# yanivw12/gs2mesh

Measured on AMD Instinct MI355X. Metric: stereo-pair renders/sec + TSDF Mvoxel-updates/sec, higher is better.
Workload: dtype f32

## Files before the change

gs2mesh_amd/_lib.py:

```python
from __future__ import annotations

import ctypes as C

import numpy as np
import os

try:
    import torch
except Exception:
    torch = None

_HERE = os.path.dirname(os.path.abspath(__file__))
LIB_PATH = os.path.join(_HERE, "libgs2mesh_amd.so")

vp = C.c_void_p
i32 = C.c_int
i64 = C.c_int64
f32 = C.c_float
f64 = C.c_double


class Camera(C.Structure):
    _fields_ = [("width", C.c_int32), ("height", C.c_int32), ("tanfovx", f32), ("tanfovy", f32),
                ("viewmatrix", f32 * 16), ("projmatrix", f32 * 16), ("campos", f32 * 3)]
# ... 73 lines not shown
    "gs2m_photo_loss_scratch_bytes": (i64, [i32, i32, i32]),
    "gs2m_photo_loss_forward": (i32, [i32, i32, i32, vp, vp, f32, vp, i64, vp, vp, vp, vp]),
    "gs2m_photo_loss_backward": (i32, [i32, i32, i32, vp, vp, vp, f32, vp, vp, vp]),
    "gs2m_adam_step": (i32, [i32, C.POINTER(AdamSegment), vp, i64, vp]),
    "gs2m_densify_stats": (i32, [i32, vp, vp, vp, vp, vp, vp]),
    "gs2m_mask_preprocess": (i32, [i32, i32, i32, C.POINTER(vp), C.POINTER(vp), i32, i32, i32, i32, C.POINTER(vp), vp, vp]),
    "gs2m_tsdf_create": (i32, [C.POINTER(vp), f64, f64, i32, i32, i32, i64, i32]),
    "gs2m_tsdf_destroy": (i32, [vp]),
    "gs2m_tsdf_reset": (i32, [vp, vp]),
    "gs2m_tsdf_integrate": (i32, [vp, vp, vp, vp, i32, i32, f64, f64, f64, f64, C.POINTER(f64), f64, f64, f64, vp]),
    "gs2m_tsdf_integrate_batch": (i32, [vp, i32, C.POINTER(vp), C.POINTER(vp), C.POINTER(vp), i32, i32, f64, f64, f64, f64,
                                        C.POINTER(f64), f64, f64, f64, vp]),
    "gs2m_tsdf_set_stage_timing": (i32, [vp, i32]),
    "gs2m_tsdf_stage_times": (i32, [vp, vp, C.POINTER(f64), C.POINTER(i64)]),
    "gs2m_tsdf_status": (i32, [vp, vp, C.POINTER(i64), C.POINTER(i64), C.POINTER(i32)]),
    "gs2m_tsdf_download": (i32, [vp, vp, i64, vp, vp, vp, vp]),
    "gs2m_tsdf_block_keys": (i32, [vp, i64, vp, vp]),
    "gs2m_tsdf_flags_device": (i32, [vp, vp, vp]),
    "gs2m_tsdf_pack_sum": (i32, [vp, vp, i64, vp, vp]),
    "gs2m_tsdf_unpack_sum": (i32, [vp, vp, i64, vp, i32, vp]),
    "gs2m_tsdf_pack": (i32, [vp, vp, i64, i32, vp, vp, vp]),
    "gs2m_tsdf_extract_mesh": (i32, [vp, vp, C.POINTER(i64), C.POINTER(i64)]),
    "gs2m_tsdf_mesh_copy": (i32, [vp, vp, vp, vp, vp, vp]),
    "gs2m_mesh_cluster": (i32, [i32, vp, i64, vp, vp, vp, C.POINTER(i64)]),
    "gs2m_mesh_vertex_normals": (i32, [i32, vp, i64, vp, i64, vp, vp, vp]),
    "gs2m_tsdf_replace": (i32, [vp, vp, i64, i32, vp, vp, vp]),
    "gs2m_tsdf_map_bytes": (i64, [C.POINTER(C.c_int32), i32]),
    "gs2m_tsdf_block_map": (i32, [vp, C.POINTER(C.c_int32), C.POINTER(C.c_int32), i32, i32, i64, i64, i32, vp, vp]),
    "gs2m_tsdf_map_keys": (i32, [vp, C.POINTER(C.c_int32), C.POINTER(C.c_int32), i32, vp, vp, i64, C.POINTER(C.c_uint8), vp]),
    "gs2m_tsdf_unpack": (i32, [vp, vp, i64, i32, vp, vp, i32, vp]),
# ... 130 lines not shown
```

gs2mesh_amd/csrc/tsdf_api.hip:

```cpp
#include <math.h>
#include <stdio.h>
#include <string.h>

#include <mutex>
#include <vector>

#include "../../include/gs2mesh_amd.h"
#include "device_memory.h"
#include "tsdf_common.h"
#include "tsdf_internal.h"

struct gs2m_tsdf {
    int device = 0;
    double voxel_length = 0, sdf_trunc = 0, unit_length = 0;
    int color_type = 1, resolution = 16, stride = 4;
    TsdfVolume V;
    struct {
        DeviceBuffer<float> tsdf, weight;
        DeviceBuffer<unsigned> rgb, stamp, touched, counters;
        DeviceBuffer<int> block_keys, hash_vals;
        DeviceBuffer<unsigned char> halo;
        DeviceBuffer<unsigned long long> hash_keys, fmask, totals;
    } vol;
    unsigned frame_id = 0;
    PinnedBuffer<unsigned> h_counters;
    PinnedBuffer<unsigned long long> h_totals;
    int n_cu = 256;
    DeviceBuffer<unsigned char> d_mc;
    const McDevTables* mc() const { return reinterpret_cast<const McDevTables*>(d_mc.get()); }
    DeviceBuffer<unsigned> d_blk_tris;
    DeviceBuffer<unsigned long long> d_ntri;
    DeviceBuffer<double> mesh_v, mesh_c;
    DeviceBuffer<int> mesh_e;
    DeviceBuffer<int> mesh_tri;
    int64_t mesh_nv = 0, mesh_nt = 0;
    ScratchArena mesh_scratch;
    int timing = 0;
// ... 39 lines not shown
    TsdfVolume& V = t->V;
    if (whole_pool) {
        GS2M_HIPCHK(hipMemsetAsync(V.tsdf, 0, sizeof(float) * (size_t)V.max_blocks * GS2M_TSDF_VOX, st));
        GS2M_HIPCHK(hipMemsetAsync(V.weight, 0, sizeof(float) * (size_t)V.max_blocks * GS2M_TSDF_VOX, st));
        if (V.rgb) GS2M_HIPCHK(hipMemsetAsync(V.rgb, 0, sizeof(unsigned) * 3 * (size_t)V.max_blocks * GS2M_TSDF_VOX, st));
        GS2M_HIPCHK(hipMemsetAsync(V.halo, 0, (size_t)V.max_blocks, st));
    } else if (keep_first < 0) {
        gs2m_launch_tsdf_clear_used(st, V);
    } else {
        gs2m_launch_tsdf_clear_from(st, V, (unsigned)keep_first);
    }
    GS2M_HIPCHK(hipMemsetAsync(V.hash_keys, 0xff, sizeof(unsigned long long) * (size_t)V.hash_cap, st));
    GS2M_HIPCHK(hipMemsetAsync(V.hash_vals, 0xff, sizeof(int) * (size_t)V.hash_cap, st));
    GS2M_HIPCHK(hipMemsetAsync(V.stamp, 0, sizeof(unsigned) * (size_t)V.hash_cap, st));
    GS2M_HIPCHK(hipMemsetAsync(V.fmask, 0, sizeof(unsigned long long) * (size_t)V.hash_cap, st));
    GS2M_HIPCHK(hipMemsetAsync(V.counters, 0, sizeof(unsigned) * 4, st));
    GS2M_HIPCHK(hipMemsetAsync(V.totals, 0, sizeof(unsigned long long), st));
    return 0;
}

static int init_volume(gs2m_tsdf* t, int64_t max_blocks) {
    memset(&t->V, 0, sizeof(t->V));
    TsdfVolume& V = t->V;
    V.max_blocks = (unsigned)max_blocks;
    unsigned cap = 1024;
    while ((uint64_t)cap < 2ull * (uint64_t)max_blocks) cap <<= 1;
    V.hash_cap = cap;
    V.has_color = t->color_type == GS2M_TSDF_COLOR_RGB8;
    const size_t nvox = (size_t)max_blocks * GS2M_TSDF_VOX, nb = (size_t)max_blocks;
    auto& o = t->vol;
    if (o.tsdf.reserve_exact(nvox) || o.weight.reserve_exact(nvox) || (V.has_color && o.rgb.reserve_exact(3 * nvox)) ||
        o.block_keys.reserve_exact(3 * nb) || o.halo.reserve_exact(nb) || o.hash_keys.reserve_exact(cap) ||
        o.hash_vals.reserve_exact(cap) || o.stamp.reserve_exact(cap) || o.touched.reserve_exact(cap) || o.fmask.reserve_exact(cap) ||
        t->d_bframes.reserve_exact(GS2M_TSDF_MAX_BATCH) || t->h_bframes.reserve(GS2M_TSDF_MAX_BATCH * gs2m_tsdf::kRing) ||
        o.counters.reserve_exact(4) || o.totals.reserve_exact(1) || t->d_mc.reserve_exact(gs2m_mc_tables_bytes()) ||
        t->d_blk_tris.reserve_exact(nb) || t->d_ntri.reserve_exact(1) || t->h_counters.reserve(4) || t->h_totals.reserve(1)) {
        gs2m_set_error("gs2m_tsdf_create: out of device memory for %lld blocks (%.1f MiB)", (long long)max_blocks,
                       (double)nvox * 20.0 / 1048576.0);
        return 1;
    }
    V.tsdf = o.tsdf.get();
    V.weight = o.weight.get();
    V.rgb = o.rgb.get();
    V.block_keys = o.block_keys.get();
    V.halo = o.halo.get();
    V.hash_keys = o.hash_keys.get();
    V.hash_vals = o.hash_vals.get();
    V.stamp = o.stamp.get();
    V.touched = o.touched.get();
    V.fmask = o.fmask.get();
    V.counters = o.counters.get();
    V.totals = o.totals.get();
    std::vector<unsigned char> tab(gs2m_mc_tables_bytes());
    if (!gs2m_mc_tables_fill(tab.data()) ||
        hipMemcpy(t->d_mc.get(), tab.data(), tab.size(), hipMemcpyHostToDevice) != hipSuccess) {
        gs2m_set_error("gs2m_tsdf_create: marching-cubes table generation failed");
        return 1;
    }
    if (zero_state(t, (hipStream_t)0, true)) return 1;
    GS2M_HIPCHK(hipStreamSynchronize((hipStream_t)0));
    return 0;
}

extern "C" int gs2m_tsdf_create(gs2m_tsdf** out, double voxel_length, double sdf_trunc, int color_type,
                                int volume_unit_resolution, int depth_sampling_stride, int64_t max_blocks,
                                int device) {
    if (!out) {
// ... 157 lines not shown
            const int i = f0 + k;
            if (!depth[i] || (t->V.has_color && !color[i])) {
                gs2m_set_error("gs2m_tsdf_integrate_batch: frame %d has a NULL image", i);
                return 1;
            }
            const unsigned char* m = mask ? mask[i] : nullptr;
            if (fill_frame(t, hb[k].f, width, height, fx, fy, cx, cy, extrinsics_w2c + 16 * (size_t)i, depth_scale, depth_trunc,
                           min_depth, m != nullptr))
                return 1;
            hb[k].depth = depth[i];
            hb[k].color = color ? color[i] : nullptr;
            hb[k].mask = m;
        }
        GS2M_HIPCHK(hipMemcpyAsync(t->d_bframes.get(), hb, sizeof(TsdfBatchFrame) * nf, hipMemcpyHostToDevice, st));
        GS2M_HIPCHK(hipEventRecord(t->ring_done[slot], st));
        GS2M_HIPCHK(hipMemsetAsync(t->V.counters + 1, 0, sizeof(unsigned), st));
        GS2M_HIPCHK(hipMemsetAsync(t->V.counters + 3, 0, sizeof(unsigned), st));
        {
            StageTimer tm(t->events, t->timing != 0, st, 0, "gs2m:tsdf_touch_batch", nf);
            gs2m_launch_tsdf_touch_batch(st, t->V, hb[0].f, nf, t->d_bframes.get(), t->d_tiles.get());
        }
        {
            StageTimer tm(t->events, t->timing != 0, st, 1, "gs2m:tsdf_integrate_batch", nf);
            gs2m_launch_tsdf_integrate_batch(st, t->n_cu, t->V, t->d_bframes.get(), t->d_tiles.get());
        }
    }
    return 0;
}

extern "C" int gs2m_tsdf_set_stage_timing(gs2m_tsdf* t, int enable) {
    if (!t) {
        gs2m_set_error("null handle");
// ... 17 lines not shown
                                int* overflow) {
    if (!t) {
        gs2m_set_error("null handle");
        return 1;
    }
    hipStream_t st = (hipStream_t)stream;
    GS2M_HIPCHK(hipMemcpyAsync(t->h_counters.get(), t->V.counters, sizeof(unsigned) * 4, hipMemcpyDeviceToHost, st));
    GS2M_HIPCHK(hipMemcpyAsync(t->h_totals.get(), t->V.totals, sizeof(unsigned long long), hipMemcpyDeviceToHost, st));
    GS2M_HIPCHK(hipStreamSynchronize(st));
    GS2M_HIPCHK(hipGetLastError());
    unsigned nb = t->h_counters.get()[0];
    if (nb > t->V.max_blocks) nb = t->V.max_blocks;
    if (n_blocks) *n_blocks = nb;
    if (block_updates) *block_updates = (int64_t)t->h_totals.get()[0];
    if (overflow) *overflow = (int)t->h_counters.get()[2];
    return 0;
}

extern "C" int gs2m_tsdf_flags_device(gs2m_tsdf* t, uint32_t* flags_dev, gs2m_stream stream) {
    if (!t || !flags_dev) {
        gs2m_set_error("gs2m_tsdf_flags_device: NULL argument");
        return 1;
    }
    GS2M_HIPCHK(hipSetDevice(t->device));
    GS2M_HIPCHK(hipMemcpyAsync(flags_dev, t->V.counters + 2, sizeof(unsigned), hipMemcpyDeviceToDevice, (hipStream_t)stream));
    return 0;
}

extern "C" int gs2m_tsdf_block_keys(gs2m_tsdf* t, int64_t n, int32_t* keys, gs2m_stream stream) {
    if (!t || (n > 0 && !keys) || n < 0 || n > (int64_t)t->V.max_blocks) {
// ... 410 lines not shown
```

gs2mesh_amd/csrc/tsdf_common.h:

```cpp
#pragma once
#include "platform.h"

#define GS2M_TSDF_RES 16
#define GS2M_TSDF_VOX 4096
#define GS2M_TSDF_EMPTY 0xffffffffffffffffull
#define GS2M_TSDF_KEY_BIAS (1 << 20)

struct TsdfVolume {
    float* tsdf;
    float* weight;
    unsigned* rgb;
    int* block_keys;
    unsigned char* halo;
    unsigned long long* hash_keys;
    int* hash_vals;
    unsigned* stamp;
    unsigned* touched;
    unsigned long long* fmask;
    unsigned* counters;
    unsigned long long* totals;
    unsigned hash_cap;
    unsigned max_blocks;
    int has_color;
};

struct alignas(16) TsdfFrame {
    float E[12];
    double pose[12];
    double fx, fy, cx, cy;
    double unit_length, sdf_trunc, depth_trunc;
    float fx_f, fy_f, cx_f, cy_f, fx_inv_f, fy_inv_f;
    float voxel_length_f, half_voxel_length_f, sdf_trunc_f, sdf_trunc_inv_f;
    float Es02, Es12, Es22;
    float safe_w, safe_h;
    float depth_scale_f, min_depth_f;
    float depth_trunc_up_f;
    int W, H, stride, nx, ny;
    unsigned frame_id;
    int use_mask, use_min;
};

struct TsdfBatchFrame {
    TsdfFrame f;
    const float* depth;
    const unsigned char* color;
    const unsigned char* mask;
};
#define GS2M_TSDF_MAX_BATCH 64
#define GS2M_TSDF_TILE 8
#define GS2M_TSDF_TILES(n) (((n) + GS2M_TSDF_TILE - 1) / GS2M_TSDF_TILE)
#define GS2M_TSDF_CULL_MAX_TILES 48

#define GS2M_TSDF_VINDEX(x, y, z) (((((z) >> 2) * 16 + ((x) >> 2) * 4 + ((y) >> 2)) * 64) + ((z)&3) * 16 + ((x)&3) * 4 + ((y)&3))

GS2M_DEVICE unsigned long long tsdf_pack_key(int bx, int by, int bz) {
    return ((unsigned long long)(unsigned)(bx + GS2M_TSDF_KEY_BIAS) << 42) |
           ((unsigned long long)(unsigned)(by + GS2M_TSDF_KEY_BIAS) << 21) |
           (unsigned long long)(unsigned)(bz + GS2M_TSDF_KEY_BIAS);
}
GS2M_DEVICE void tsdf_unpack_key(unsigned long long key, int& bx, int& by, int& bz) {
    bx = (int)((key >> 42) & 0x1fffffull) - GS2M_TSDF_KEY_BIAS;
    by = (int)((key >> 21) & 0x1fffffull) - GS2M_TSDF_KEY_BIAS;
// ... 15 lines not shown
```

gs2mesh_amd/csrc/tsdf_internal.h:

```cpp
#pragma once
#include "api_check.h"
#include "tsdf_common.h"

void gs2m_launch_tsdf_touch(hipStream_t st, const TsdfVolume& V, const TsdfFrame& f, const float* depth,
                            const unsigned char* mask);
void gs2m_launch_tsdf_integrate(hipStream_t st, int n_wg, const TsdfVolume& V, const TsdfFrame& f,
                                const float* depth, const unsigned char* color, const unsigned char* mask);
void gs2m_launch_tsdf_touch_batch(hipStream_t st, const TsdfVolume& V, const TsdfFrame& f, int n_frames,
                                  const TsdfBatchFrame* frames, float* tiles);
void gs2m_launch_tsdf_integrate_batch(hipStream_t st, int n_wg, const TsdfVolume& V, const TsdfBatchFrame* frames, const float* tiles);
void gs2m_launch_tsdf_clear_used(hipStream_t st, const TsdfVolume& V);
void gs2m_launch_tsdf_pack(hipStream_t st, unsigned n, const TsdfVolume& V, const int* keys, int form, float* buf, long long* ibuf);
void gs2m_launch_tsdf_unpack(hipStream_t st, unsigned n, const TsdfVolume& V, const int* keys, int form, const float* buf,
                             const long long* ibuf, int halo);
void gs2m_launch_tsdf_clear_from(hipStream_t st, const TsdfVolume& V, unsigned first);
void gs2m_launch_tsdf_clear_gap(hipStream_t st, const TsdfVolume& V, unsigned upto);
void gs2m_launch_tsdf_owned_keys(hipStream_t st, unsigned n, const TsdfVolume& V, int* keys);
void gs2m_launch_tsdf_block_map(hipStream_t st, const TsdfVolume& V, const int* lo, const int* dim, unsigned char* cells, unsigned n_cells,
                                unsigned flags, unsigned win_hash, int rank, unsigned frames_local, unsigned frames_base);
void gs2m_launch_tsdf_map_keys(hipStream_t st, const int* lo, const int* dim, unsigned char* cells, unsigned n_cells, int* keys, unsigned max_keys);
struct McDevTables;
size_t gs2m_mc_tables_bytes();
bool gs2m_mc_tables_fill(void* host_buf);
void gs2m_launch_mc_count(hipStream_t st, const TsdfVolume& V, const McDevTables* T, unsigned n_blocks,
                          unsigned* blk_tris, unsigned long long* n_total);
// ... 18 lines not shown
```

gs2mesh_amd/csrc/tsdf_kernels.h:

```cpp
#pragma once
#include "tsdf_common.h"


GS2M_DEVICE void tsdf_cam_point(const TsdfFrame& f, float p0, float p1, float p2, float& pc0, float& pc1, float& pc2) {
    pc0 = f.E[0] * p0 + f.E[1] * p1 + f.E[2] * p2 + f.E[3] * 1.f;
    pc1 = f.E[4] * p0 + f.E[5] * p1 + f.E[6] * p2 + f.E[7] * 1.f;
    pc2 = f.E[8] * p0 + f.E[9] * p1 + f.E[10] * p2 + f.E[11] * 1.f;
}
GS2M_DEVICE void tsdf_z_step(const TsdfFrame& f, float& pc0, float& pc1, float& pc2) {
    pc0 += f.Es02;
    pc1 += f.Es12;
    pc2 += f.Es22;
}
GS2M_DEVICE int tsdf_project(const TsdfFrame& f, float pc0, float pc1, float pc2, int& u, int& v) {
    if (pc2 <= 0) return -1;
    const float u_f = pc0 * f.fx_f / pc2 + f.cx_f + 0.5f;
    const float v_f = pc1 * f.fy_f / pc2 + f.cy_f + 0.5f;
    if (!(u_f >= 0.0001f && u_f < f.safe_w && v_f >= 0.0001f && v_f < f.safe_h)) return -1;
    u = (int)u_f;
    v = (int)v_f;
    return v * f.W + u;
}
GS2M_DEVICE float tsdf_distance_multiplier(const TsdfFrame& f, int u, int v) {
    const float xx = (u - f.cx_f) * f.fx_inv_f;
// ... 20 lines not shown
    return d > 0.0f && sdf > -f.sdf_trunc_f;
}
GS2M_DEVICE unsigned tsdf_gather_rgb(const unsigned char* __restrict__ color, int pix, int last_pix) {
    const unsigned char* c = color + 3 * (size_t)pix;
    return pix < last_pix ? gs2m_load_u32_unaligned(c) : ((unsigned)c[0] | ((unsigned)c[1] << 8) | ((unsigned)c[2] << 16));
}
GS2M_DEVICE void tsdf_update_mean(float& t, float& w, float tnew) {
    t = (t * w + tnew) / (w + 1.0f);
    w = w + 1.0f;
}
GS2M_DEVICE void tsdf_update_rgb(unsigned& c0, unsigned& c1, unsigned& c2, unsigned rgbp) {
    c0 += rgbp & 0xffu;
    c1 += (rgbp >> 8) & 0xffu;
    c2 += (rgbp >> 16) & 0xffu;
}
GS2M_DEVICE float tsdf_block_centres(const TsdfFrame& f, unsigned long long key, int tid, float* s_p0, float* s_p1) {
    int bx, by, bz;
    tsdf_unpack_key(key, bx, by, bz);
    const double ox = (double)bx * f.unit_length, oy = (double)by * f.unit_length, oz = (double)bz * f.unit_length;
    if (tid < 16) s_p0[tid] = (float)(f.half_voxel_length_f + f.voxel_length_f * tid + ox);
    else if (tid < 32) s_p1[tid - 16] = (float)(f.half_voxel_length_f + f.voxel_length_f * (tid - 16) + oy);
    return (float)(f.half_voxel_length_f + oz);
}

GS2M_DEVICE unsigned tsdf_find_or_insert(const TsdfVolume& V, unsigned long long key, int bx, int by, int bz) {
    const unsigned mask = V.hash_cap - 1u;
    unsigned h = tsdf_hash(key) & mask;
    for (unsigned probe = 0; probe < V.hash_cap; ++probe, h = (h + 1u) & mask) {
        unsigned long long k = V.hash_keys[h];
        if (k == key) return h;
        if (k == GS2M_TSDF_EMPTY) {
            const unsigned long long prev = atomicCAS(&V.hash_keys[h], GS2M_TSDF_EMPTY, key);
            if (prev == GS2M_TSDF_EMPTY) {
                const unsigned slot = atomicAdd(&V.counters[0], 1u);
                if (slot < V.max_blocks) {
                    V.block_keys[3 * (size_t)slot] = bx;
// ... 303 lines not shown
        }
#pragma unroll
        for (int s = 1; s < GS2M_TSDF_TILE; s <<= 1) {
            const float o = gs2m_shfl_xor(m, s);
            if (o > m) m = o;
        }
        if ((lane & (GS2M_TSDF_TILE - 1)) == 0 && x < f.W) out[x / GS2M_TSDF_TILE] = m;
    }
}

GS2M_KERNEL void __launch_bounds__(256)
k_tsdf_touch_batch(TsdfVolume V, const TsdfBatchFrame* __restrict__ frames, unsigned n_touch, float* __restrict__ tiles, int tiles_x,
                   int tiles_y, unsigned map_wg_x) {
    __shared__ TouchStage stage_all[4];
    const TsdfBatchFrame& bf = frames[blockIdx.y];
    if (blockIdx.x < n_touch) {
        tsdf_touch_body(V, bf.f, bf.depth, bf.mask, stage_all, (int)blockIdx.y);
    } else {
        const unsigned m = blockIdx.x - n_touch, ty = m / map_wg_x;
        tsdf_depth_tiles_body(bf, tiles + ((size_t)blockIdx.y * tiles_y + ty) * tiles_x, (int)(m - ty * map_wg_x), (int)ty);
    }
}

GS2M_DEVICE bool tsdf_pass_live(const TsdfFrame& f0, const float4* __restrict__ e4, const float* __restrict__ tiles, int tiles_x,
                                float xa, float xb, float ya, float yb, float z0) {
    const float4 r0 = e4[0], r1 = e4[1], r2 = e4[2];
    const float vl = f0.voxel_length_f, zspan = 15.0f * vl;
    const float ax = fmaxf(fabsf(xa), fabsf(xb)), ay = fmaxf(fabsf(ya), fabsf(yb)), az = fabsf(z0) + zspan + vl;
    const float S = fmaxf(fmaxf(fabsf(r0.x) * ax + fabsf(r0.y) * ay + fabsf(r0.z) * az + fabsf(r0.w),
                                fabsf(r1.x) * ax + fabsf(r1.y) * ay + fabsf(r1.z) * az + fabsf(r1.w)),
                          fabsf(r2.x) * ax + fabsf(r2.y) * ay + fabsf(r2.z) * az + fabsf(r2.w));
    const float eps = S * (1.0f / 262144.0f);
    const float bx = r0.x * xa + r0.y * ya + r0.z * z0 + r0.w, by = r1.x * xa + r1.y * ya + r1.z * z0 + r1.w,
                bz = r2.x * xa + r2.y * ya + r2.z * z0 + r2.w;
    const float dx[3] = {r0.x * (xb - xa), r0.y * (yb - ya), r0.z * zspan};
    const float dy[3] = {r1.x * (xb - xa), r1.y * (yb - ya), r1.z * zspan};
    const float dz[3] = {r2.x * (xb - xa), r2.y * (yb - ya), r2.z * zspan};
    float cx[8], cy[8], cz[8], zmin = bz;
// ... 17 lines not shown
        vmax = fmaxf(vmax, v);
        mag += fabsf(u) + fabsf(v);
    }
    if (!(mag < 1e9f)) return true;
    const float au = fmaxf(fabsf(umin), fabsf(umax)), av = fmaxf(fabsf(vmin), fabsf(vmax));
    const float k = eps / zl, rnd = 1.0f / 1048576.0f;
    const float mu = 1.0f + k * (fabsf(f0.fx_f) + au) + rnd * (au + fabsf(f0.cx_f) + 1.0f);
    const float mv = 1.0f + k * (fabsf(f0.fy_f) + av) + rnd * (av + fabsf(f0.cy_f) + 1.0f);
    if (!(mu < 1e6f && mv < 1e6f)) return true;
    const float x0 = fmaxf(floorf(umin + f0.cx_f - mu), 0.0f), x1 = fminf(ceilf(umax + f0.cx_f + mu), (float)(f0.W - 1));
    const float y0 = fmaxf(floorf(vmin + f0.cy_f - mv), 0.0f), y1 = fminf(ceilf(vmax + f0.cy_f + mv), (float)(f0.H - 1));
    if (x0 > x1 || y0 > y1) return false;
    const int tx0 = (int)x0 / GS2M_TSDF_TILE, tx1 = (int)x1 / GS2M_TSDF_TILE, ty0 = (int)y0 / GS2M_TSDF_TILE, ty1 = (int)y1 / GS2M_TSDF_TILE;
    if ((tx1 - tx0 + 1) * (ty1 - ty0 + 1) > GS2M_TSDF_CULL_MAX_TILES) return true;
    float dmax = 0.0f;
    for (int ty = ty0; ty <= ty1; ty += 4) {
        for (int tx = tx0; tx <= tx1; tx += 4) {
            float d[16];
#pragma unroll
            for (int i = 0; i < 4; ++i) {
                const float* __restrict__ row = tiles + (size_t)(ty + i < ty1 ? ty + i : ty1) * tiles_x;
#pragma unroll
                for (int j = 0; j < 4; ++j) d[4 * i + j] = row[tx + j < tx1 ? tx + j : tx1];
            }
#pragma unroll
            for (int i = 0; i < 16; ++i)
                if (d[i] > dmax) dmax = d[i];
        }
    }
    if (!(dmax > 0.0f)) return false;
    const float zlow = zl - vl;
    return !(dmax - zlow <= -f0.sdf_trunc_f);
}

GS2M_KERNEL void __launch_bounds__(256)
k_tsdf_integrate_batch(TsdfVolume V, const TsdfBatchFrame* __restrict__ frames, const float* __restrict__ tiles) {
    __shared__ float s_p0[16], s_p1[16];
    const int tid = (int)threadIdx.x;
    const int lane = tid & 63, wave = tid >> 6;
    const int lz = lane >> 4, lx = (lane >> 2) & 3, ly = lane & 3;
    __shared__ unsigned s_it;
    const unsigned n_touched = V.counters[1] * 4u;
    const TsdfFrame& f0 = frames[0].f;
    for (;;) {
        __syncthreads();
        if (tid == 0) s_it = atomicAdd(&V.counters[3], 1u);
        __syncthreads();
        const unsigned it = s_it;
        if (it >= n_touched) break;
        const int xq = (int)(it & 3u);
        const unsigned h = V.touched[it >> 2];
        const unsigned long long key = V.hash_keys[h];
        const int slot = V.hash_vals[h];
        const unsigned long long fm = V.fmask[h];
        if (slot < 0) continue;
        const float p2 = tsdf_block_centres(f0, key, tid, s_p0, s_p1);
        __syncthreads();
        const float p0 = s_p0[4 * xq + lx], p1 = s_p1[4 * wave + ly];
        const int vi0 = (xq * 4 + wave) * 64 + lane;
        constexpr int VS = 16 * 64;
        float* bt = V.tsdf + (size_t)slot * GS2M_TSDF_VOX;
        float* bw = V.weight + (size_t)slot * GS2M_TSDF_VOX;
        unsigned* bc = V.rgb + (size_t)slot * 3 * GS2M_TSDF_VOX;
        bool live = false;
        if ((fm >> lane) & 1ull) {
            const int tiles_x = GS2M_TSDF_TILES(f0.W), tiles_y = GS2M_TSDF_TILES(f0.H);
            live = tsdf_pass_live(f0, reinterpret_cast<const float4*>(frames[lane].f.E), tiles + (size_t)lane * tiles_y * tiles_x, tiles_x,
                                  s_p0[4 * xq], s_p0[4 * xq + 3], s_p1[4 * wave], s_p1[4 * wave + 3], p2);
        }
        const unsigned long long fm_live = fm & gs2m_ballot(live ? 1 : 0);
        float w[4], t[4];
        unsigned c0[4], c1[4], c2[4];
#pragma unroll
        for (int j = 0; j < 4; ++j) {
            w[j] = t[j] = 0.0f;
            c0[j] = c1[j] = c2[j] = 0u;
            if (fm_live != 0ull) {
                w[j] = bw[vi0 + VS * j];
                t[j] = bt[vi0 + VS * j];
                if (V.has_color) {
                    c0[j] = bc[vi0 + VS * j];
                    c1[j] = bc[GS2M_TSDF_VOX + vi0 + VS * j];
                    c2[j] = bc[2 * GS2M_TSDF_VOX + vi0 + VS * j];
                }
            }
// ... 85 lines not shown
                if (todo == 0ull) break;
            }
            apply(A);
        }
#pragma unroll
        for (int j = 0; j < 4; ++j) {
            if (fm_live == 0ull) continue;
            bw[vi0 + VS * j] = w[j];
            bt[vi0 + VS * j] = t[j];
            if (V.has_color) {
                bc[vi0 + VS * j] = c0[j];
                bc[GS2M_TSDF_VOX + vi0 + VS * j] = c1[j];
                bc[2 * GS2M_TSDF_VOX + vi0 + VS * j] = c2[j];
            }
        }
        if (tid == 0 && xq == 0) atomicAdd(&V.totals[0], (unsigned long long)gs2m_popc64(fm));
    }
}

GS2M_KERNEL void __launch_bounds__(256)
k_tsdf_clear_fmask(TsdfVolume V) {
    const unsigned n = V.counters[1];
    for (unsigned i = blockIdx.x * 256u + threadIdx.x; i < n; i += gridDim.x * 256u) V.fmask[V.touched[i]] = 0ull;
}

GS2M_KERNEL void __launch_bounds__(256)
k_tsdf_clear_used(TsdfVolume V) {
    unsigned n = V.counters[0];
    if (n > V.max_blocks) n = V.max_blocks;
    const float4 z = {0.f, 0.f, 0.f, 0.f};
    for (unsigned slot = blockIdx.x; slot < n; slot += gridDim.x) {
        float4* t4 = reinterpret_cast<float4*>(V.tsdf + (size_t)slot * GS2M_TSDF_VOX);
        float4* w4 = reinterpret_cast<float4*>(V.weight + (size_t)slot * GS2M_TSDF_VOX);
        for (int i = (int)threadIdx.x; i < GS2M_TSDF_VOX / 4; i += 256) {
            t4[i] = z;
            w4[i] = z;
        }
        if (V.has_color) {
// ... 223 lines not shown
```

gs2mesh_amd/csrc/tsdf_kernels.hip:

```cpp
#include "tsdf_kernels.h"
#include "tsdf_extract.h"
#include "mesh_kernels.h"
#include "tsdf_internal.h"
#include <math.h>

void gs2m_launch_tsdf_touch(hipStream_t st, const TsdfVolume& V, const TsdfFrame& f, const float* depth,
                            const unsigned char* mask) {
    const int n = f.nx * f.ny;
    GS2M_LAUNCH(k_tsdf_touch, dim3((n + 255) / 256), dim3(256), 0, st, V, f, depth, mask);
    GS2M_LAUNCH(k_tsdf_compact, dim3((V.hash_cap + 1023u) / 1024u), dim3(1024), 0, st, V, f.frame_id);
}
void gs2m_launch_tsdf_integrate(hipStream_t st, int n_wg, const TsdfVolume& V, const TsdfFrame& f,
                                const float* depth, const unsigned char* color, const unsigned char* mask) {
    GS2M_LAUNCH(k_tsdf_integrate, dim3(n_wg), dim3(256), 0, st, V, f, depth, color, mask);
}
void gs2m_launch_tsdf_touch_batch(hipStream_t st, const TsdfVolume& V, const TsdfFrame& f, int n_frames,
                                  const TsdfBatchFrame* frames, float* tiles) {
    const int n = f.nx * f.ny;
    const int tiles_x = GS2M_TSDF_TILES(f.W), tiles_y = GS2M_TSDF_TILES(f.H);
    const unsigned n_touch = (unsigned)((n + 255) / 256), map_wg_x = (unsigned)((f.W + 1023) / 1024);
    GS2M_LAUNCH(k_tsdf_touch_batch, dim3(n_touch + map_wg_x * (unsigned)tiles_y, n_frames), dim3(256), 0, st, V, frames, n_touch, tiles, tiles_x,
                tiles_y, map_wg_x);
    GS2M_LAUNCH(k_tsdf_compact, dim3((V.hash_cap + 1023u) / 1024u), dim3(1024), 0, st, V, 0u);
}
void gs2m_launch_tsdf_integrate_batch(hipStream_t st, int n_cu, const TsdfVolume& V, const TsdfBatchFrame* frames, const float* tiles) {
    GS2M_LAUNCH(k_tsdf_integrate_batch, dim3(n_cu * 6), dim3(256), 0, st, V, frames, tiles);
    GS2M_LAUNCH(k_tsdf_clear_fmask, dim3(16), dim3(256), 0, st, V);
}
void gs2m_launch_tsdf_clear_used(hipStream_t st, const TsdfVolume& V) {
    GS2M_LAUNCH(k_tsdf_clear_used, dim3(2048), dim3(256), 0, st, V);
}
void gs2m_launch_tsdf_pack(hipStream_t st, unsigned n, const TsdfVolume& V, const int* keys, int form, float* buf, long long* ibuf) {
    if (form == GS2M_XF_SUM_PACKED) GS2M_LAUNCH(k_tsdf_pack<GS2M_XF_SUM_PACKED>, dim3(n), dim3(256), 0, st, V, keys, buf, ibuf);
    else if (form == GS2M_XF_RAW_F32) GS2M_LAUNCH(k_tsdf_pack<GS2M_XF_RAW_F32>, dim3(n), dim3(256), 0, st, V, keys, buf, ibuf);
    else GS2M_LAUNCH(k_tsdf_pack<GS2M_XF_SUM_F32>, dim3(n), dim3(256), 0, st, V, keys, buf, ibuf);
}
void gs2m_launch_tsdf_unpack(hipStream_t st, unsigned n, const TsdfVolume& V, const int* keys, int form, const float* buf,
                             const long long* ibuf, int halo) {
    if (form == GS2M_XF_SUM_PACKED) GS2M_LAUNCH(k_tsdf_unpack<GS2M_XF_SUM_PACKED>, dim3(n), dim3(256), 0, st, V, keys, buf, ibuf, halo);
    else if (form == GS2M_XF_RAW_F32) GS2M_LAUNCH(k_tsdf_unpack<GS2M_XF_RAW_F32>, dim3(n), dim3(256), 0, st, V, keys, buf, ibuf, halo);
    else GS2M_LAUNCH(k_tsdf_unpack<GS2M_XF_SUM_F32>, dim3(n), dim3(256), 0, st, V, keys, buf, ibuf, halo);
}
// ... 93 lines not shown
```

gs2mesh_amd/integration.py:

```python
from __future__ import annotations

import ctypes as C
import enum

import numpy as np

from . import _lib
from ._lib import _is_torch, _ptr, _stream_of

try:
    import torch
except Exception:
    torch = None


class TSDFVolumeColorType(enum.IntEnum):
    NoColor = 0
    RGB8 = 1
    Gray32 = 2


class PinholeCameraIntrinsic:
    def __init__(self, width, height, fx, fy, cx, cy):
        self.width, self.height = int(width), int(height)
# ... 153 lines not shown
        if len(self._keep) > 64:
            self.status(stream)

    def status(self, stream=None, raise_on_overflow=True):
        nb, bu, ov = C.c_int64(0), C.c_int64(0), C.c_int(0)
        _lib.check(self._lib.gs2m_tsdf_status(self._h, stream or C.c_void_p(0), C.byref(nb), C.byref(bu),
                                              C.byref(ov)), self._lib)
        self._keep.clear()
        if ov.value and raise_on_overflow:
            what = [n for b, n in ((1, "block pool exhausted (raise max_blocks)"), (2, "hash table full"),
                                   (4, "block index out of the +-2^20 range"),
                                   (8, "a voxel did not fit the packed exchange form (weight > 1023: use payload='f32')")) if ov.value & b]
            raise RuntimeError("TSDF volume overflow: " + ", ".join(what))
        return int(nb.value), int(bu.value), int(ov.value)

    def set_stage_timing(self, enable=True):
        _lib.check(self._lib.gs2m_tsdf_set_stage_timing(self._h, int(bool(enable))), self._lib)

    def stage_times(self, stream=None):
        ms = (C.c_double * 2)()
        cnt = (C.c_int64 * 2)()
        _lib.check(self._lib.gs2m_tsdf_stage_times(self._h, stream or C.c_void_p(0), ms, cnt), self._lib)
        return {name: (ms[i], cnt[i]) for i, name in enumerate(_lib.TSDF_STAGES)}

    @property
    def num_blocks(self):
        return self.status()[0]

    @property
    def voxel_updates(self):
# ... 115 lines not shown
```

include/gs2mesh_amd.h:

```cpp
#ifndef GS2MESH_AMD_H
#define GS2MESH_AMD_H

#include <stddef.h>
#include <stdint.h>

#ifdef __cplusplus
extern "C" {
#endif

#define GS2M_VERSION 600

typedef void* gs2m_stream;


int gs2m_version(void);
const char* gs2m_last_error(void);


typedef struct gs2m_raster gs2m_raster;

enum {
    GS2M_OPT_EXACT_TILE_CULL = 1,
    GS2M_OPT_BLEND_VARIANT = 2,
    GS2M_OPT_DEBUG_SYNC = 3,
// ... 120 lines not shown
int gs2m_tsdf_integrate(gs2m_tsdf* t, const float* depth, const uint8_t* color,
                        const uint8_t* mask, int width, int height, double fx, double fy,
                        double cx, double cy, const double* extrinsic_w2c, double depth_scale,
                        double depth_trunc, double min_depth, gs2m_stream stream);

int gs2m_tsdf_integrate_batch(gs2m_tsdf* t, int n_frames, const float* const* depth, const uint8_t* const* color,
                              const uint8_t* const* mask, int width, int height, double fx, double fy, double cx,
                              double cy, const double* extrinsics_w2c, double depth_scale, double depth_trunc,
                              double min_depth, gs2m_stream stream);

int gs2m_tsdf_set_stage_timing(gs2m_tsdf* t, int enable);
int gs2m_tsdf_stage_times(gs2m_tsdf* t, gs2m_stream stream, double* total_ms, int64_t* launches);

int gs2m_tsdf_status(gs2m_tsdf* t, gs2m_stream stream, int64_t* n_blocks,
                     int64_t* block_updates, int* overflow);

int gs2m_tsdf_flags_device(gs2m_tsdf* t, uint32_t* flags_dev, gs2m_stream stream);

int gs2m_tsdf_download(gs2m_tsdf* t, gs2m_stream stream, int64_t n, int32_t* keys,
                       float* tsdf, float* weight, uint32_t* rgb_sum);

int gs2m_tsdf_block_keys(gs2m_tsdf* t, int64_t n, int32_t* keys, gs2m_stream stream);

int gs2m_tsdf_pack_sum(gs2m_tsdf* t, const int32_t* keys, int64_t n, float* buf, gs2m_stream stream);
int gs2m_tsdf_unpack_sum(gs2m_tsdf* t, const int32_t* keys, int64_t n, const float* buf, int halo,
                         gs2m_stream stream);

#define GS2M_TSDF_MAP_HEADER_BYTES 32
int64_t gs2m_tsdf_map_bytes(const int32_t* dim, int world);
int gs2m_tsdf_block_map(gs2m_tsdf* t, const int32_t* lo, const int32_t* dim, int rank, int world, int64_t frames_local,
// ... 103 lines not shown
```

Baseline: 4268.

## Split TSDF batch integration into a frame-liveness plan pass and integrate pass

Adds a planning kernel that, per touched block and x-quarter, evaluates frame liveness culling in parallel across 16 lanes per frame-chunk and writes a compact plan item (key, slot, per-wave live masks). The integrate kernel reads the plan, skips block quarters with no live frames before computing centres, and drops its own per-lane culling and the separate fmask-clear kernel. Counter resets move from host memsets into the touch kernel, and the tile max scan uses unaligned 4-wide loads. It adds an extra kernel launch and a plan buffer of four items per hash slot, plus a diagnostic plan-count API.

```diff
diff --git a/gs2mesh_amd/_lib.py b/gs2mesh_amd/_lib.py
--- a/gs2mesh_amd/_lib.py
+++ b/gs2mesh_amd/_lib.py
@@ -111,6 +111,7 @@
     "gs2m_tsdf_set_stage_timing": (i32, [vp, i32]),
     "gs2m_tsdf_stage_times": (i32, [vp, vp, C.POINTER(f64), C.POINTER(i64)]),
     "gs2m_tsdf_status": (i32, [vp, vp, C.POINTER(i64), C.POINTER(i64), C.POINTER(i32)]),
+    "gs2m_tsdf_plan_counts": (i32, [vp, vp, C.POINTER(i64), C.POINTER(i64)]),
     "gs2m_tsdf_download": (i32, [vp, vp, i64, vp, vp, vp, vp]),
     "gs2m_tsdf_block_keys": (i32, [vp, i64, vp, vp]),
     "gs2m_tsdf_flags_device": (i32, [vp, vp, vp]),
diff --git a/gs2mesh_amd/csrc/tsdf_api.hip b/gs2mesh_amd/csrc/tsdf_api.hip
--- a/gs2mesh_amd/csrc/tsdf_api.hip
+++ b/gs2mesh_amd/csrc/tsdf_api.hip
@@ -21,6 +21,7 @@
         DeviceBuffer<int> block_keys, hash_vals;
         DeviceBuffer<unsigned char> halo;
         DeviceBuffer<unsigned long long> hash_keys, fmask, totals;
+        DeviceBuffer<TsdfPlanItem> plan;
     } vol;
     unsigned frame_id = 0;
     PinnedBuffer<unsigned> h_counters;
@@ -90,8 +91,8 @@
     GS2M_HIPCHK(hipMemsetAsync(V.hash_vals, 0xff, sizeof(int) * (size_t)V.hash_cap, st));
     GS2M_HIPCHK(hipMemsetAsync(V.stamp, 0, sizeof(unsigned) * (size_t)V.hash_cap, st));
     GS2M_HIPCHK(hipMemsetAsync(V.fmask, 0, sizeof(unsigned long long) * (size_t)V.hash_cap, st));
-    GS2M_HIPCHK(hipMemsetAsync(V.counters, 0, sizeof(unsigned) * 4, st));
-    GS2M_HIPCHK(hipMemsetAsync(V.totals, 0, sizeof(unsigned long long), st));
+    GS2M_HIPCHK(hipMemsetAsync(V.counters, 0, sizeof(unsigned) * GS2M_TSDF_COUNTERS, st));
+    GS2M_HIPCHK(hipMemsetAsync(V.totals, 0, sizeof(unsigned long long) * GS2M_TSDF_TOTALS, st));
     return 0;
 }
 
@@ -109,8 +110,9 @@
         o.block_keys.reserve_exact(3 * nb) || o.halo.reserve_exact(nb) || o.hash_keys.reserve_exact(cap) ||
         o.hash_vals.reserve_exact(cap) || o.stamp.reserve_exact(cap) || o.touched.reserve_exact(cap) || o.fmask.reserve_exact(cap) ||
         t->d_bframes.reserve_exact(GS2M_TSDF_MAX_BATCH) || t->h_bframes.reserve(GS2M_TSDF_MAX_BATCH * gs2m_tsdf::kRing) ||
-        o.counters.reserve_exact(4) || o.totals.reserve_exact(1) || t->d_mc.reserve_exact(gs2m_mc_tables_bytes()) ||
-        t->d_blk_tris.reserve_exact(nb) || t->d_ntri.reserve_exact(1) || t->h_counters.reserve(4) || t->h_totals.reserve(1)) {
+        o.counters.reserve_exact(GS2M_TSDF_COUNTERS) || o.totals.reserve_exact(GS2M_TSDF_TOTALS) ||
+        o.plan.reserve_exact(4 * (size_t)cap) || t->d_mc.reserve_exact(gs2m_mc_tables_bytes()) ||
+        t->d_blk_tris.reserve_exact(nb) || t->d_ntri.reserve_exact(1) || t->h_counters.reserve(4) || t->h_totals.reserve(GS2M_TSDF_TOTALS)) {
         gs2m_set_error("gs2m_tsdf_create: out of device memory for %lld blocks (%.1f MiB)", (long long)max_blocks,
                        (double)nvox * 20.0 / 1048576.0);
         return 1;
@@ -127,6 +129,7 @@
     V.fmask = o.fmask.get();
     V.counters = o.counters.get();
     V.totals = o.totals.get();
+    V.plan = o.plan.get();
     std::vector<unsigned char> tab(gs2m_mc_tables_bytes());
     if (!gs2m_mc_tables_fill(tab.data()) ||
         hipMemcpy(t->d_mc.get(), tab.data(), tab.size(), hipMemcpyHostToDevice) != hipSuccess) {
@@ -314,8 +317,6 @@
         }
         GS2M_HIPCHK(hipMemcpyAsync(t->d_bframes.get(), hb, sizeof(TsdfBatchFrame) * nf, hipMemcpyHostToDevice, st));
         GS2M_HIPCHK(hipEventRecord(t->ring_done[slot], st));
-        GS2M_HIPCHK(hipMemsetAsync(t->V.counters + 1, 0, sizeof(unsigned), st));
-        GS2M_HIPCHK(hipMemsetAsync(t->V.counters + 3, 0, sizeof(unsigned), st));
         {
             StageTimer tm(t->events, t->timing != 0, st, 0, "gs2m:tsdf_touch_batch", nf);
             gs2m_launch_tsdf_touch_batch(st, t->V, hb[0].f, nf, t->d_bframes.get(), t->d_tiles.get());
@@ -363,6 +364,22 @@
     if (n_blocks) *n_blocks = nb;
     if (block_updates) *block_updates = (int64_t)t->h_totals.get()[0];
     if (overflow) *overflow = (int)t->h_counters.get()[2];
+    return 0;
+}
+
+extern "C" int gs2m_tsdf_plan_counts(gs2m_tsdf* t, gs2m_stream stream, int64_t* planned, int64_t* dropped) {
+    if (!t) {
+        gs2m_set_error("null handle");
+        return 1;
+    }
+    GS2M_HIPCHK(hipSetDevice(t->device));
+    hipStream_t st = (hipStream_t)stream;
+    GS2M_HIPCHK(hipMemsetAsync(t->V.totals + 1, 0, sizeof(unsigned long long) * 2, st));
+    gs2m_launch_tsdf_plan_count(st, t->V);
+    GS2M_HIPCHK(hipMemcpyAsync(t->h_totals.get(), t->V.totals, sizeof(unsigned long long) * GS2M_TSDF_TOTALS, hipMemcpyDeviceToHost, st));
+    GS2M_HIPCHK(hipStreamSynchronize(st));
+    if (planned) *planned = (int64_t)t->h_totals.get()[1];
+    if (dropped) *dropped = (int64_t)t->h_totals.get()[2];
     return 0;
 }
 
diff --git a/gs2mesh_amd/csrc/tsdf_common.h b/gs2mesh_amd/csrc/tsdf_common.h
--- a/gs2mesh_amd/csrc/tsdf_common.h
+++ b/gs2mesh_amd/csrc/tsdf_common.h
@@ -19,6 +19,7 @@
     unsigned long long* fmask;
     unsigned* counters;
     unsigned long long* totals;
+    struct TsdfPlanItem* plan;
     unsigned hash_cap;
     unsigned max_blocks;
     int has_color;
@@ -46,6 +47,14 @@
     const unsigned char* color;
     const unsigned char* mask;
 };
+struct alignas(16) TsdfPlanItem {
+    unsigned long long key;
+    int slot;
+    unsigned n_frames;
+    unsigned long long live[4];
+};
+#define GS2M_TSDF_COUNTERS 8
+#define GS2M_TSDF_TOTALS 3
 #define GS2M_TSDF_MAX_BATCH 64
 #define GS2M_TSDF_TILE 8
 #define GS2M_TSDF_TILES(n) (((n) + GS2M_TSDF_TILE - 1) / GS2M_TSDF_TILE)
diff --git a/gs2mesh_amd/csrc/tsdf_internal.h b/gs2mesh_amd/csrc/tsdf_internal.h
--- a/gs2mesh_amd/csrc/tsdf_internal.h
+++ b/gs2mesh_amd/csrc/tsdf_internal.h
@@ -9,6 +9,7 @@
 void gs2m_launch_tsdf_touch_batch(hipStream_t st, const TsdfVolume& V, const TsdfFrame& f, int n_frames,
                                   const TsdfBatchFrame* frames, float* tiles);
 void gs2m_launch_tsdf_integrate_batch(hipStream_t st, int n_wg, const TsdfVolume& V, const TsdfBatchFrame* frames, const float* tiles);
+void gs2m_launch_tsdf_plan_count(hipStream_t st, const TsdfVolume& V);
 void gs2m_launch_tsdf_clear_used(hipStream_t st, const TsdfVolume& V);
 void gs2m_launch_tsdf_pack(hipStream_t st, unsigned n, const TsdfVolume& V, const int* keys, int form, float* buf, long long* ibuf);
 void gs2m_launch_tsdf_unpack(hipStream_t st, unsigned n, const TsdfVolume& V, const int* keys, int form, const float* buf,
diff --git a/gs2mesh_amd/csrc/tsdf_kernels.h b/gs2mesh_amd/csrc/tsdf_kernels.h
--- a/gs2mesh_amd/csrc/tsdf_kernels.h
+++ b/gs2mesh_amd/csrc/tsdf_kernels.h
@@ -58,12 +58,15 @@
     c1 += (rgbp >> 8) & 0xffu;
     c2 += (rgbp >> 16) & 0xffu;
 }
+GS2M_DEVICE float tsdf_block_centre(const TsdfFrame& f, int i, double origin) {
+    return (float)(f.half_voxel_length_f + f.voxel_length_f * i + origin);
+}
 GS2M_DEVICE float tsdf_block_centres(const TsdfFrame& f, unsigned long long key, int tid, float* s_p0, float* s_p1) {
     int bx, by, bz;
     tsdf_unpack_key(key, bx, by, bz);
     const double ox = (double)bx * f.unit_length, oy = (double)by * f.unit_length, oz = (double)bz * f.unit_length;
-    if (tid < 16) s_p0[tid] = (float)(f.half_voxel_length_f + f.voxel_length_f * tid + ox);
-    else if (tid < 32) s_p1[tid - 16] = (float)(f.half_voxel_length_f + f.voxel_length_f * (tid - 16) + oy);
+    if (tid < 16) s_p0[tid] = tsdf_block_centre(f, tid, ox);
+    else if (tid < 32) s_p1[tid - 16] = tsdf_block_centre(f, tid - 16, oy);
     return (float)(f.half_voxel_length_f + oz);
 }
 
@@ -397,6 +400,7 @@
                    int tiles_y, unsigned map_wg_x) {
     __shared__ TouchStage stage_all[4];
     const TsdfBatchFrame& bf = frames[blockIdx.y];
+    if (blockIdx.x == 0 && blockIdx.y == 0 && threadIdx.x == 0) V.counters[1] = V.counters[3] = 0u;
     if (blockIdx.x < n_touch) {
         tsdf_touch_body(V, bf.f, bf.depth, bf.mask, stage_all, (int)blockIdx.y);
     } else {
@@ -405,6 +409,9 @@
     }
 }
 
+struct __attribute__((packed, aligned(4))) TsdfTileQuad {
+    float v[4];
+};
 GS2M_DEVICE bool tsdf_pass_live(const TsdfFrame& f0, const float4* __restrict__ e4, const float* __restrict__ tiles, int tiles_x,
                                 float xa, float xb, float ya, float yb, float z0) {
     const float4 r0 = e4[0], r1 = e4[1], r2 = e4[2];
@@ -452,18 +459,37 @@
     const int tx0 = (int)x0 / GS2M_TSDF_TILE, tx1 = (int)x1 / GS2M_TSDF_TILE, ty0 = (int)y0 / GS2M_TSDF_TILE, ty1 = (int)y1 / GS2M_TSDF_TILE;
     if ((tx1 - tx0 + 1) * (ty1 - ty0 + 1) > GS2M_TSDF_CULL_MAX_TILES) return true;
     float dmax = 0.0f;
-    for (int ty = ty0; ty <= ty1; ty += 4) {
-        for (int tx = tx0; tx <= tx1; tx += 4) {
-            float d[16];
-#pragma unroll
-            for (int i = 0; i < 4; ++i) {
-                const float* __restrict__ row = tiles + (size_t)(ty + i < ty1 ? ty + i : ty1) * tiles_x;
-#pragma unroll
-                for (int j = 0; j < 4; ++j) d[4 * i + j] = row[tx + j < tx1 ? tx + j : tx1];
-            }
-#pragma unroll
-            for (int i = 0; i < 16; ++i)
-                if (d[i] > dmax) dmax = d[i];
+    if (tiles_x >= 4) {
+        for (int ty = ty0; ty <= ty1; ty += 4) {
+            for (int tx = tx0; tx <= tx1; tx += 4) {
+                const int ts = tx < tiles_x - 4 ? tx : tiles_x - 4;
+                TsdfTileQuad q[4];
+#pragma unroll
+                for (int i = 0; i < 4; ++i)
+                    q[i] = *reinterpret_cast<const TsdfTileQuad*>(tiles + (size_t)(ty + i < ty1 ? ty + i : ty1) * tiles_x + ts);
+#pragma unroll
+                for (int j = 0; j < 4; ++j) {
+                    const bool in = ts + j >= tx && ts + j <= tx1;
+#pragma unroll
+                    for (int i = 0; i < 4; ++i)
+                        if (in && q[i].v[j] > dmax) dmax = q[i].v[j];
+                }
+            }
+        }
+    } else {
+        for (int ty = ty0; ty <= ty1; ty += 4) {
+            for (int tx = tx0; tx <= tx1; tx += 4) {
+                float d[16];
+#pragma unroll
+                for (int i = 0; i < 4; ++i) {
+                    const float* __restrict__ row = tiles + (size_t)(ty + i < ty1 ? ty + i : ty1) * tiles_x;
+#pragma unroll
+                    for (int j = 0; j < 4; ++j) d[4 * i + j] = row[tx + j < tx1 ? tx + j : tx1];
+                }
+#pragma unroll
+                for (int i = 0; i < 16; ++i)
+                    if (d[i] > dmax) dmax = d[i];
+            }
         }
     }
     if (!(dmax > 0.0f)) return false;
@@ -472,26 +498,96 @@
 }
 
 GS2M_KERNEL void __launch_bounds__(256)
-k_tsdf_integrate_batch(TsdfVolume V, const TsdfBatchFrame* __restrict__ frames, const float* __restrict__ tiles) {
+k_tsdf_plan_batch(TsdfVolume V, const TsdfBatchFrame* __restrict__ frames, const float* __restrict__ tiles) {
+    const int lane = (int)(threadIdx.x & 63u), xq = gs2m_uniform((int)(threadIdx.x >> 6));
+    const int yq = lane >> 4, jl = lane & 15;
+    const unsigned n_touched = V.counters[1];
+    const TsdfFrame& f0 = frames[0].f;
+    const int tiles_x = GS2M_TSDF_TILES(f0.W), tiles_y = GS2M_TSDF_TILES(f0.H);
+    if (blockIdx.x == 0 && threadIdx.x == 0) V.counters[4] = n_touched * 4u;
+    for (unsigned it = blockIdx.x; it < n_touched; it += gridDim.x) {
+        const unsigned h = V.touched[it];
+        const int slot = V.hash_vals[h];
+        const unsigned long long key = V.hash_keys[h], fm = V.fmask[h];
+        __syncthreads();
+        if (threadIdx.x == 0) V.fmask[h] = 0ull;
+        unsigned long long mine = 0ull;
+        if (slot >= 0) {
+            int bx, by, bz;
+            tsdf_unpack_key(key, bx, by, bz);
+            const double ox = (double)bx * f0.unit_length, oy = (double)by * f0.unit_length, oz = (double)bz * f0.unit_length;
+            const float xa = tsdf_block_centre(f0, 4 * xq, ox), xb = tsdf_block_centre(f0, 4 * xq + 3, ox);
+            const float ya = tsdf_block_centre(f0, 4 * yq, oy), yb = tsdf_block_centre(f0, 4 * yq + 3, oy);
+            const float p2 = (float)(f0.half_voxel_length_f + oz);
+            unsigned long long todo = fm;
+            while (todo != 0ull) {
+                int fi = -1;
+                for (int j = 0; j < 16 && todo != 0ull; ++j) {
+                    const int b = __ffsll(todo) - 1;
+                    todo &= todo - 1ull;
+                    if (j == jl) fi = b;
+                }
+                unsigned lo = 0u, hi = 0u;
+                if (fi >= 0 && tsdf_pass_live(f0, reinterpret_cast<const float4*>(frames[fi].f.E), tiles + (size_t)fi * tiles_y * tiles_x, tiles_x,
+                                              xa, xb, ya, yb, p2)) {
+                    lo = fi < 32 ? 1u << fi : 0u;
+                    hi = fi < 32 ? 0u : 1u << (fi - 32);
+                }
+#pragma unroll
+                for (int s = 1; s < 16; s <<= 1) {
+                    lo |= gs2m_shfl_xor(lo, s);
+                    hi |= gs2m_shfl_xor(hi, s);
+                }
+                mine |= (unsigned long long)lo | ((unsigned long long)hi << 32);
+            }
+        }
+        TsdfPlanItem item;
+        item.key = key;
+        item.slot = slot;
+        item.n_frames = slot >= 0 ? (unsigned)gs2m_popc64(fm) : 0u;
+#pragma unroll
+        for (int y = 0; y < 4; ++y) item.live[y] = gs2m_shfl(mine, 16 * y);
+        if (lane == 0) V.plan[(size_t)it * 4 + xq] = item;
+    }
+}
+
+GS2M_KERNEL void __launch_bounds__(1024)
+k_tsdf_plan_count(TsdfVolume V) {
+    const unsigned n = V.counters[4];
+    unsigned planned = 0u, dropped = 0u;
+    for (unsigned i = blockIdx.x * 1024u + threadIdx.x; i < n; i += gridDim.x * 1024u) {
+        const TsdfPlanItem& item = V.plan[i];
+        if (item.slot < 0) continue;
+        if ((item.live[0] | item.live[1] | item.live[2] | item.live[3]) != 0ull) ++planned;
+        else ++dropped;
+    }
+    if (planned) atomicAdd(&V.totals[1], (unsigned long long)planned);
+    if (dropped) atomicAdd(&V.totals[2], (unsigned long long)dropped);
+}
+
+GS2M_KERNEL void __launch_bounds__(256)
+k_tsdf_integrate_batch(TsdfVolume V, const TsdfBatchFrame* __restrict__ frames, const TsdfPlanItem* __restrict__ plan) {
     __shared__ float s_p0[16], s_p1[16];
     const int tid = (int)threadIdx.x;
     const int lane = tid & 63, wave = tid >> 6;
     const int lz = lane >> 4, lx = (lane >> 2) & 3, ly = lane & 3;
     __shared__ unsigned s_it;
-    const unsigned n_touched = V.counters[1] * 4u;
+    const unsigned n_items = V.counters[1] * 4u;
     const TsdfFrame& f0 = frames[0].f;
     for (;;) {
         __syncthreads();
         if (tid == 0) s_it = atomicAdd(&V.counters[3], 1u);
         __syncthreads();
-        const unsigned it = s_it;
-        if (it >= n_touched) break;
+        const unsigned it = (unsigned)gs2m_uniform((int)s_it);
+        if (it >= n_items) break;
+        const TsdfPlanItem& item = plan[it];
         const int xq = (int)(it & 3u);
-        const unsigned h = V.touched[it >> 2];
-        const unsigned long long key = V.hash_keys[h];
-        const int slot = V.hash_vals[h];
-        const unsigned long long fm = V.fmask[h];
-        if (slot < 0) continue;
+        const unsigned long long key = item.key;
+        const int slot = item.slot;
+        const unsigned n_upd = item.n_frames;
+        const unsigned long long live_any = item.live[0] | item.live[1] | item.live[2] | item.live[3];
+        if (tid == 0 && xq == 0) atomicAdd(&V.totals[0], (unsigned long long)n_upd);
+        if (live_any == 0ull) continue;
         const float p2 = tsdf_block_centres(f0, key, tid, s_p0, s_p1);
         __syncthreads();
         const float p0 = s_p0[4 * xq + lx], p1 = s_p1[4 * wave + ly];
@@ -500,13 +596,7 @@
         float* bt = V.tsdf + (size_t)slot * GS2M_TSDF_VOX;
         float* bw = V.weight + (size_t)slot * GS2M_TSDF_VOX;
         unsigned* bc = V.rgb + (size_t)slot * 3 * GS2M_TSDF_VOX;
-        bool live = false;
-        if ((fm >> lane) & 1ull) {
-            const int tiles_x = GS2M_TSDF_TILES(f0.W), tiles_y = GS2M_TSDF_TILES(f0.H);
-            live = tsdf_pass_live(f0, reinterpret_cast<const float4*>(frames[lane].f.E), tiles + (size_t)lane * tiles_y * tiles_x, tiles_x,
-                                  s_p0[4 * xq], s_p0[4 * xq + 3], s_p1[4 * wave], s_p1[4 * wave + 3], p2);
-        }
-        const unsigned long long fm_live = fm & gs2m_ballot(live ? 1 : 0);
+        const unsigned long long fm_live = item.live[gs2m_uniform(wave)];
         float w[4], t[4];
         unsigned c0[4], c1[4], c2[4];
 #pragma unroll
@@ -622,14 +712,7 @@
                 bc[2 * GS2M_TSDF_VOX + vi0 + VS * j] = c2[j];
             }
         }
-        if (tid == 0 && xq == 0) atomicAdd(&V.totals[0], (unsigned long long)gs2m_popc64(fm));
-    }
-}
-
-GS2M_KERNEL void __launch_bounds__(256)
-k_tsdf_clear_fmask(TsdfVolume V) {
-    const unsigned n = V.counters[1];
-    for (unsigned i = blockIdx.x * 256u + threadIdx.x; i < n; i += gridDim.x * 256u) V.fmask[V.touched[i]] = 0ull;
+    }
 }
 
 GS2M_KERNEL void __launch_bounds__(256)
diff --git a/gs2mesh_amd/csrc/tsdf_kernels.hip b/gs2mesh_amd/csrc/tsdf_kernels.hip
--- a/gs2mesh_amd/csrc/tsdf_kernels.hip
+++ b/gs2mesh_amd/csrc/tsdf_kernels.hip
@@ -24,8 +24,11 @@
     GS2M_LAUNCH(k_tsdf_compact, dim3((V.hash_cap + 1023u) / 1024u), dim3(1024), 0, st, V, 0u);
 }
 void gs2m_launch_tsdf_integrate_batch(hipStream_t st, int n_cu, const TsdfVolume& V, const TsdfBatchFrame* frames, const float* tiles) {
-    GS2M_LAUNCH(k_tsdf_integrate_batch, dim3(n_cu * 6), dim3(256), 0, st, V, frames, tiles);
-    GS2M_LAUNCH(k_tsdf_clear_fmask, dim3(16), dim3(256), 0, st, V);
+    GS2M_LAUNCH(k_tsdf_plan_batch, dim3(n_cu * 8), dim3(256), 0, st, V, frames, tiles);
+    GS2M_LAUNCH(k_tsdf_integrate_batch, dim3(n_cu * 6), dim3(256), 0, st, V, frames, V.plan);
+}
+void gs2m_launch_tsdf_plan_count(hipStream_t st, const TsdfVolume& V) {
+    GS2M_LAUNCH(k_tsdf_plan_count, dim3(16), dim3(1024), 0, st, V);
 }
 void gs2m_launch_tsdf_clear_used(hipStream_t st, const TsdfVolume& V) {
     GS2M_LAUNCH(k_tsdf_clear_used, dim3(2048), dim3(256), 0, st, V);
diff --git a/gs2mesh_amd/integration.py b/gs2mesh_amd/integration.py
--- a/gs2mesh_amd/integration.py
+++ b/gs2mesh_amd/integration.py
@@ -191,6 +191,11 @@
             raise RuntimeError("TSDF volume overflow: " + ", ".join(what))
         return int(nb.value), int(bu.value), int(ov.value)
 
+    def plan_counts(self, stream=None):
+        planned, dropped = C.c_int64(0), C.c_int64(0)
+        _lib.check(self._lib.gs2m_tsdf_plan_counts(self._h, stream or C.c_void_p(0), C.byref(planned), C.byref(dropped)), self._lib)
+        return int(planned.value), int(dropped.value)
+
     def set_stage_timing(self, enable=True):
         _lib.check(self._lib.gs2m_tsdf_set_stage_timing(self._h, int(bool(enable))), self._lib)
 
diff --git a/include/gs2mesh_amd.h b/include/gs2mesh_amd.h
--- a/include/gs2mesh_amd.h
+++ b/include/gs2mesh_amd.h
@@ -158,6 +158,8 @@
 
 int gs2m_tsdf_status(gs2m_tsdf* t, gs2m_stream stream, int64_t* n_blocks,
                      int64_t* block_updates, int* overflow);
+
+int gs2m_tsdf_plan_counts(gs2m_tsdf* t, gs2m_stream stream, int64_t* planned, int64_t* dropped);
 
 int gs2m_tsdf_flags_device(gs2m_tsdf* t, uint32_t* flags_dev, gs2m_stream stream);
 
```

Result: no change. 4287 (median of 6 runs) (+0.4%).
